# lgw-frank/Short_LDPC_Decoding_OSD

Hardware: AMD Instinct MI355X
Metric: decoded frames/sec + FER, (128,64) LDPC NMS-10+OSD-2 @ 2.5 dB (higher is better)
Workload: dtype f32; 1 GPU; nms10_osd2 -- configs[3]: NMS-10 + OSD-2, 2^20 frames over 8 GPUs = 131 072 per GPU; code=CCSDS (128,64), osd_order=2, frames_per_gpu=131072, parallelism=frame-sharded x1, rccl_ranks=1, distinct_batches_per_gpu=4, distinct_frames=524288, bytes_in_plus_out_per_rotation=545783808, nms_kernel=qc16, streams=1, osd_route=front+search

## Files before the change

### short_ldpc_decoding_osd_amd/csrc/ldpc_front.h

```cpp
#pragma once
#include "ldpc_internal.h"
#include "ldpc_wave.h"

namespace ldpc {

struct __attribute__((aligned(16))) FrontLds {
    RankLds rank;
    u64 colbuf[64];
    unsigned mask[4];
    unsigned char pi1[128];
    unsigned char rowsrc[64];
    unsigned char perm[128];
};

struct FrontResult {
    int o1, o2;
    u64 Prow;
    int ns;
};


__device__ __forceinline__ FrontResult front_device_vals(FrontLds &L, unsigned a1, unsigned a2, const u64 *__restrict__ Gcols, int lane)
{
    const float bs = bucket_scale(a1, a2);
    int r1, r2;
    bucket_ranks(L.rank, ((u64)a1 << 32) | (unsigned)(127 - lane), ((u64)a2 << 32) | (unsigned)(63 - lane), bucket_of(a1, bs),
                 bucket_of(a2, bs), lane, r1, r2);
    L.pi1[r1] = (unsigned char)lane;
    L.pi1[r2] = (unsigned char)(lane + 64);
    if (lane < 4) L.mask[lane] = 0;
    wave_fence();
    u64 C1 = Gcols[L.pi1[lane]];
    u64 C2 = Gcols[L.pi1[lane + 64]];
    int rho = lane, idx1 = lane, idx2 = lane + 64;
    const int ns = ge_columns(C1, C2, rho, idx1, idx2, lane, nullptr);
    int rankM = lane, rankL = lane;
    if (ns != 0) {
        atomicOr(&L.mask[idx1 >> 5], 1u << (idx1 & 31));
        wave_fence();
        const unsigned m[4] = {L.mask[0], L.mask[1], L.mask[2], L.mask[3]};
        rankM = below_mask(m, idx1);
        rankL = idx2 - below_mask(m, idx2);
    }
    L.perm[rankM] = L.pi1[idx1];
    L.perm[64 + rankL] = L.pi1[idx2];
    L.colbuf[rankL] = C2;
    L.rowsrc[rankM] = (unsigned char)rho;
    wave_fence();
    const u64 R = transpose64(L.colbuf[lane], lane);
    FrontResult res;
    res.Prow = shfl64(R, L.rowsrc[lane]);
    res.o1 = L.perm[lane];
    res.o2 = L.perm[64 + lane];
    res.ns = ns;
    wave_fence();
    return res;
}

__device__ __forceinline__ FrontResult front_device(FrontLds &L, const float *__restrict__ y, long long src,
                                                    const u64 *__restrict__ Gcols, int lane)
{
    return front_device_vals(L, __float_as_uint(y[src * 128 + lane]) & 0x7FFFFFFFu, __float_as_uint(y[src * 128 + 64 + lane]) & 0x7FFFFFFFu, Gcols, lane);
}


}
```

### short_ldpc_decoding_osd_amd/csrc/ldpc_osd.hip

```cpp
#include <math.h>
#include <stdlib.h>

#include "ldpc_osd_small.h"
#include "ldpc_osd_scan2.h"
#include "ldpc_osd_scan2r.h"
#include "ldpc_osd_fs.h"
#include "ldpc_osd_aux.h"
#include "ldpc_osd_state.h"

namespace ldpc {

int osd_ctx_init(ldpc_ctx *ctx)
{
    const OsdTables &t = ctx->osd_tables;
    ctx->osd_ok = false;
    if (t.n != kOsdN || t.k != kOsdK) return LDPC_OK;
    OsdState *st = new OsdState();
    ctx->osd_state = st;
    {
        int base2[127];
        auto npairs = [](int t) { return (t - 1) / 2 - (t > 63 ? t - 63 : 0) + 1; };
        for (int sidx = 0; sidx < 127; ++sidx) {
            int acc = 0;
            for (int t = sidx + 1; t <= 125; ++t) acc += npairs(t);
// ... 111 lines not shown

static unsigned grid2r(const ldpc_ctx *ctx, int64_t F) { const int64_t g = (int64_t)ctx->cu_count * 16 * 6; return (unsigned)(F < g ? F : g); }

static void launch_front(ldpc_ctx *ctx, const float *d_y, const int32_t *d_index, const int32_t *d_count, int64_t F, uint8_t *d_perm,
                         u64 *d_parity, int32_t *d_nswaps, hipStream_t s)
{
    hipLaunchKernelGGL(osd_front_kernel, dim3(frame_grid(F)), dim3(64), 0, s, d_y, d_index, d_count, (long long)F,
                       ctx->osd_tables.d_Gcols, d_perm, d_parity, d_nswaps);
}

static int need_osd(const ldpc_ctx *ctx)
{
    return ctx->osd_ok ? LDPC_OK : fail(LDPC_E_UNSUPPORTED, "OSD kernels need an (n=128, k=64) code; this one is (%d,%d)", ctx->code.n, ctx->code.k);
}

static const char *flag_name(unsigned f)
{
    if (f & LDPC_OSD_F_TABLE_SCAN) return "LDPC_OSD_F_TABLE_SCAN";
    if (f & LDPC_OSD_F_PB_BLOCK) return "LDPC_OSD_F_PB_BLOCK";
    if (f & LDPC_OSD_F_PB_REPLAY) return "LDPC_OSD_F_PB_REPLAY";
    if (f & LDPC_OSD_F_READLANE_SCAN) return "LDPC_OSD_F_READLANE_SCAN";
    return "LDPC_OSD_F_PB_FRONT_INSIDE";
}

int check_params(ldpc_ctx *ctx, const ldpc_osd_params *p, bool front_outside, const char *who)
{
    if (int rc = need_osd(ctx)) return rc;
    if (p->order < 0 || p->order > 3) return fail(LDPC_E_ARG, "%s: order %d outside 0..3", who, p->order);
    if (p->algo != LDPC_OSD_CONVENTIONAL && p->algo != LDPC_OSD_FS && p->algo != LDPC_OSD_PB)
        return fail(LDPC_E_ARG, "%s: unknown search algorithm %d", who, p->algo);
    if (p->algo == LDPC_OSD_PB && p->order < 1) return fail(LDPC_E_ARG, "%s: PB-OSD needs order >= 1", who);
    const unsigned f = (unsigned)p->flags;
    const unsigned conv = LDPC_OSD_F_TABLE_SCAN | LDPC_OSD_F_READLANE_SCAN;
    const unsigned pb = LDPC_OSD_F_PB_BLOCK | LDPC_OSD_F_PB_REPLAY | LDPC_OSD_F_PB_FRONT_INSIDE;
    if (f & ~(conv | pb)) return fail(LDPC_E_ARG, "%s: flags 0x%x are no LDPC_OSD_F_* flag", who, f & ~(conv | pb));
    if ((f & conv) && p->algo != LDPC_OSD_CONVENTIONAL)
        return fail(LDPC_E_ARG, "%s: %s needs the conventional algorithm, not %d", who, flag_name(f & conv), p->algo);
    if ((f & LDPC_OSD_F_READLANE_SCAN) && (p->order != 2 || (f & LDPC_OSD_F_TABLE_SCAN)))
        return fail(LDPC_E_ARG, "%s: LDPC_OSD_F_READLANE_SCAN needs order 2 (not %d) and no LDPC_OSD_F_TABLE_SCAN", who, p->order);
    if ((f & pb) && p->algo != LDPC_OSD_PB)
        return fail(LDPC_E_ARG, "%s: %s needs the PB algorithm, not %d", who, flag_name(f & pb), p->algo);
    if ((f & LDPC_OSD_F_PB_REPLAY) && (f & (LDPC_OSD_F_PB_BLOCK | LDPC_OSD_F_PB_FRONT_INSIDE)))
        return fail(LDPC_E_ARG, "%s: LDPC_OSD_F_PB_REPLAY excludes %s", who, flag_name(f & (LDPC_OSD_F_PB_BLOCK | LDPC_OSD_F_PB_FRONT_INSIDE)));
    if ((f & LDPC_OSD_F_PB_FRONT_INSIDE) && front_outside)
        return fail(LDPC_E_ARG, "%s: LDPC_OSD_F_PB_FRONT_INSIDE keeps the front-end results inside the PB kernels, and this call "
                    "supplies or wants them", who);
    return LDPC_OK;
}

OsdPlan select_route(const ldpc_ctx *ctx, const ldpc_osd_params *p, bool front_outside)
{
    const unsigned f = (unsigned)p->flags;
    if (p->algo == LDPC_OSD_FS) return {OsdRoute::Fs, 0};
    if (p->algo == LDPC_OSD_PB)
        return {(f & LDPC_OSD_F_PB_FRONT_INSIDE) ? OsdRoute::PbFrontInside : OsdRoute::PbStaged,
                (f & LDPC_OSD_F_PB_REPLAY) ? 2 : ((f & LDPC_OSD_F_PB_BLOCK) ? 1 : 0)};
    if (p->order != 2 || (f & LDPC_OSD_F_TABLE_SCAN)) return {OsdRoute::Table, 0};
    if ((f & LDPC_OSD_F_READLANE_SCAN) || ctx->dpp_wave_rol_dir == 0) return {OsdRoute::Search2, 0};
    return {front_outside ? OsdRoute::Search2r : OsdRoute::Fused2r, 0};
}

int osd_launch(ldpc_ctx *ctx, const float *d_y, const int32_t *d_index, const int32_t *d_count, int64_t F, const uint8_t *d_perm,
               const uint64_t *d_parity, const ldpc_osd_params *p, uint64_t *d_cw, float *d_metric, int32_t *d_best, int32_t *d_ntep,
               const uint64_t *d_label, int64_t *d_counts, hipStream_t s, bool *counted)
{
    *counted = false;
    const OsdPlan r = select_route(ctx, p, d_perm != nullptr);
    OsdState *st = state(ctx);
    const OsdTables &t = ctx->osd_tables;
    int rc;
    if ((rc = guarded_index(ctx, p, d_index, d_count, F, s, &d_index))) return rc;
    if (!d_perm && r.route != OsdRoute::Fused2r && r.route != OsdRoute::PbFrontInside) {
        StreamWs *w;
        if ((rc = stream_ws(ctx, s, F, &w))) return rc;
        launch_front(ctx, d_y, d_index, d_count, F, w->d_perm, w->d_parity, nullptr, s);
        d_perm = w->d_perm; d_parity = reinterpret_cast<const uint64_t *>(w->d_parity);
    }
    const u64 *const parity = reinterpret_cast<const u64 *>(d_parity);
    u64 *const cw = reinterpret_cast<u64 *>(d_cw);
    const u64 *const label = d_label && d_counts ? reinterpret_cast<const u64 *>(d_label) : nullptr;
    u64 *const counts = label ? reinterpret_cast<u64 *>(d_counts) : nullptr;
    const unsigned g2r = grid2r(ctx, F), g64 = frame_grid(F);
    switch (r.route) {
    case OsdRoute::Fused2r:
        hipLaunchKernelGGL(osd_fused2r_kernel, dim3(g2r), dim3(64), 0, s, d_y, d_index, d_count, (long long)F,
                           t.d_Gcols, ctx->dpp_wave_rol_dir, st->d_base2, cw, d_metric, d_best, d_ntep, label, counts);
        *counted = label != nullptr;
        break;
    case OsdRoute::Search2r:
        hipLaunchKernelGGL(osd_search2r_kernel, dim3(g2r), dim3(64), 0, s, d_y, d_index, d_count, (long long)F, d_perm, parity,
                           ctx->dpp_wave_rol_dir, st->d_base2, cw, d_metric, d_best, d_ntep, label, counts);
        *counted = label != nullptr;
        break;
    case OsdRoute::Search2:
        hipLaunchKernelGGL(osd_search2_kernel, dim3(g64), dim3(64), 0, s, d_y, d_index, d_count, (long long)F, d_perm, parity, st->d_base2,
                           cw, d_metric, d_best, d_ntep);
        break;
    case OsdRoute::Table:
        if (p->order >= 2)
            hipLaunchKernelGGL(osd_search_kernel<1>, dim3(g64), dim3(64), 0, s, d_y, d_index, d_count, (long long)F, d_perm, parity,
                               t.d_tep, (int)t.ntep[p->order], cw, d_metric, d_best, d_ntep);
        else
            hipLaunchKernelGGL(osd_search_kernel<4>, dim3(osd_grid(F)), dim3(256), 0, s, d_y, d_index, d_count, (long long)F, d_perm, parity,
                               t.d_tep, (int)t.ntep[p->order], cw, d_metric, d_best, d_ntep);
        break;
    case OsdRoute::Fs:
        hipLaunchKernelGGL(osd_fs_kernel, dim3(g64), dim3(64), 0, s, d_y, d_index, d_count, (long long)F, d_perm, parity, t.d_tep_fs,
                           fs_params(p, t), cw, d_metric, d_best, d_ntep);
        break;
    case OsdRoute::PbStaged:
        return launch_pb(ctx, d_y, d_index, d_count, F, d_perm, parity, p, r.pb_mode, false, d_cw, d_metric, d_best, d_ntep, s);
    case OsdRoute::PbFrontInside:
        return launch_pb(ctx, d_y, d_index, d_count, F, nullptr, nullptr, p, r.pb_mode, true, d_cw, d_metric, d_best, d_ntep, s);
    }
    LDPC_HIP(hipGetLastError());
    return LDPC_OK;
}

FsParams fs_params(const ldpc_osd_params *p, const OsdTables &t)
{
    FsParams fp;
    fp.order = p->order; fp.quirk = p->fs_reference_quirk != 0;
    fp.beta_term = (float)((double)p->fs_beta * (double)(t.n - t.k));
    fp.tau_e = p->fs_tau_e; fp.tau_psc = p->fs_tau_psc;
    for (int w = 0; w < 4; ++w) { fp.cls_off[w] = t.fs_off[w]; fp.cls_cnt[w] = t.fs_cnt[w]; }
    return fp;
}

}

using namespace ldpc;

extern "C" {

int ldpc_osd_reserve(ldpc_ctx *ctx, int64_t max_frames)
{
    if (!ctx || max_frames < 0) return fail(LDPC_E_ARG, "ldpc_osd_reserve: bad arguments");
    if (int rc = need_osd(ctx)) return rc;
    {
        OsdState *st = state(ctx);
        std::lock_guard<std::mutex> lock(st->mu);
        if (max_frames > st->reserve_frames) st->reserve_frames = max_frames;
    }
    StreamWs *w;
    return stream_ws(ctx, nullptr, max_frames, &w);
}

int ldpc_osd_reserve_stream(ldpc_ctx *ctx, int64_t max_frames, const ldpc_osd_params *params, void *stream)
{
    if (!ctx || max_frames < 0) return fail(LDPC_E_ARG, "ldpc_osd_reserve_stream: bad arguments");
    int rc;
    if ((rc = need_osd(ctx))) return rc;
    if (params && (rc = check_params(ctx, params, false, "ldpc_osd_reserve_stream"))) return rc;
    StreamWs *w;
    if ((rc = stream_ws(ctx, (hipStream_t)stream, max_frames, &w)) || !params) return rc;
    if (params->algo == LDPC_OSD_PB && max_frames > 0) return pb_reserve(ctx, (hipStream_t)stream, max_frames, params->order);
    return LDPC_OK;
}

int ldpc_osd_release_stream(ldpc_ctx *ctx, void *stream)
{
    if (!ctx) return fail(LDPC_E_ARG, "ldpc_osd_release_stream: null ctx");
    OsdState *st = state(ctx);
    if (!st) return LDPC_OK;
    if (stream_capturing((hipStream_t)stream)) return fail(LDPC_E_ARG, "ldpc_osd_release_stream: the stream is capturing");
    std::lock_guard<std::mutex> lock(st->mu);
    auto it = st->ws.find((hipStream_t)stream);
    if (it != st->ws.end()) { free_stream_ws(it->second); st->ws.erase(it); }
    return LDPC_OK;
}

int ldpc_osd_ge(ldpc_ctx *ctx, const uint64_t *d_rows_in, int64_t F, uint64_t *d_rows_out, uint8_t *d_swaps,
                int32_t *d_nswaps, void *stream)
{
    if (!ctx || F < 0 || (F > 0 && (!d_rows_in || !d_rows_out))) return fail(LDPC_E_ARG, "ldpc_osd_ge: bad arguments");
    if (int rc = need_osd(ctx)) return rc;
// ... 86 lines not shown
```

### short_ldpc_decoding_osd_amd/csrc/ldpc_osd_scan2r.h

```cpp
#pragma once

#include "ldpc_front.h"
#include "ldpc_osd_scan2.h"

namespace ldpc {

struct __attribute__((aligned(16))) Search2rLds {
    float lut[8][256];
    uint2 q[128];
    u64 P[64];
    __device__ __forceinline__ float *wpar() { return reinterpret_cast<float *>(q); }
    __device__ __forceinline__ u64 *cw() { return reinterpret_cast<u64 *>(q) + 32; }
};
static_assert(sizeof(Search2rLds) <= 10240, "LDS budget of the rotation scan");

__device__ __forceinline__ float cost2r(const Search2rLds &L, float mrb, u64 D)
{
    float acc = mrb;
    acc = acc + lut_byte<0>(L.lut, D); acc = acc + lut_byte<1>(L.lut, D); acc = acc + lut_byte<2>(L.lut, D); acc = acc + lut_byte<3>(L.lut, D);
    acc = acc + lut_byte<4>(L.lut, D); acc = acc + lut_byte<5>(L.lut, D); acc = acc + lut_byte<6>(L.lut, D); acc = acc + lut_byte<7>(L.lut, D);
    return acc;
}

__device__ __forceinline__ int wave_rot1(int x) { return __builtin_amdgcn_update_dpp(0, x, 0x134, 0xF, 0xF, true); }

__device__ __forceinline__ void search2r_finish_batch(const Search2rLds &L, uint2 e, bool valid, int dir, u64 d0, const int *__restrict__ base2,
                                                      float &best, int &bi, int &bj, u64 &bestD)
{
    if (!valid) return;
    const int r = (int)(e.y >> 6), l = (int)(e.y & 63), m = (l - dir * r) & 63;
    const u64 D = d0 ^ L.P[l] ^ L.P[m];
    float acc = __uint_as_float(e.x);
    acc = acc + lut_byte<2>(L.lut, D); acc = acc + lut_byte<3>(L.lut, D); acc = acc + lut_byte<4>(L.lut, D);
    acc = acc + lut_byte<5>(L.lut, D); acc = acc + lut_byte<6>(L.lut, D); acc = acc + lut_byte<7>(L.lut, D);
    if (!(acc <= best)) return;
    search2_take(acc, l < m ? l : m, l < m ? m : l, D, base2, best, bi, bj, bestD);
}

struct Scan2r {
    float m, t0, t1;
    float bound;
    int plo, wr;
    int qn;
};

__device__ __forceinline__ bool search2r_round(Search2rLds &LL, Scan2r &s, int R, unsigned dlo, float wl, int lane)
{
    float mn = 0.0f, u0 = 0.0f, u1 = 0.0f;
    if (R < 32) {
        s.plo = wave_rot1(s.plo); s.wr = wave_rot1(s.wr);
        const unsigned Dn = dlo ^ (unsigned)s.plo;
        mn = wl + __int_as_float(s.wr); u0 = lut_byte<0>(LL.lut, Dn); u1 = lut_byte<1>(LL.lut, Dn);
    }
    float acc = s.m + s.t0;
    acc = acc + s.t1;
    s.m = mn; s.t0 = u0; s.t1 = u1;
    const bool keep = (R < 32 || lane < 32) && !(acc > s.bound);
    const u64 km = __ballot(keep);
    if (!km) return false;
    if (keep) {
        const int slot = wave_lane_rank(km, (unsigned)s.qn);
        LL.q[slot] = make_uint2(__float_as_uint(acc), (unsigned)(R * 64 + lane));
    }
    s.qn += __popcll(km);
    return s.qn >= 64;
}

__device__ __forceinline__ void search2r_device(Search2rLds &LL, const SearchFrame &S, u64 Pl, float wl, int dir,
                                                const int *__restrict__ base2, int lane, float &best_out, int &rank_out,
                                                u64 &D_out, u64 &E_out)
{
    Search2rLds &L = LL;
    LL.P[lane] = Pl;
    float best;
    int bi, bj;
    u64 bestD;
    search2_start([&](float mrb, u64 D) { return cost2r(L, mrb, D); }, S.d0, Pl, wl, lane, best, bi, bj, bestD);
    const unsigned dlo = (unsigned)(S.d0 ^ Pl);
    Scan2r s;
    s.bound = wave_min_f32(best);
    s.qn = 0;
    s.plo = wave_rot1((int)(unsigned)Pl); s.wr = wave_rot1(__float_as_int(wl));
    s.m = wl + __int_as_float(s.wr);
    s.t0 = lut_byte<0>(L.lut, dlo ^ (unsigned)s.plo); s.t1 = lut_byte<1>(L.lut, dlo ^ (unsigned)s.plo);
#pragma unroll
    for (int r = 1; r <= 32; ++r) {
        if (search2r_round(LL, s, r, dlo, wl, lane)) {
            wave_fence();
            const uint2 e = LL.q[lane], rest = LL.q[64 + lane];
            s.qn -= 64;
            if (lane < s.qn) LL.q[lane] = rest;
            search2r_finish_batch(L, e, true, dir, S.d0, base2, best, bi, bj, bestD);
            s.bound = wave_min_f32(best);
            wave_fence();
        }
    }
    wave_fence();
    search2r_finish_batch(L, LL.q[lane], lane < s.qn, dir, S.d0, base2, best, bi, bj, bestD);
    wave_fence();
    int bestt = tep2_rank(bi, bj, base2);
    u64 bestE = (bi >= 0 ? 1ull << bi : 0ull) | (bj >= 0 ? 1ull << bj : 0ull);
    wave_argmin(best, bestt, bestD, bestE, lane);
    best_out = best; rank_out = bestt; D_out = bestD; E_out = bestE;
}

__device__ __forceinline__ void search2r_frame(Search2rLds &LL, int o1, int o2, u64 Pl, float y1, float y2, int dir, const int *base2,
                                               long long f, u64 lab, int lane, u64 *cw_out, float *metric_out, int *best_out,
                                               int *ntep_out, u64 *counts)
{
    SearchFrame S;
    S.o1 = o1; S.o2 = o2;
    const float w1 = __builtin_fabsf(y1), w2 = __builtin_fabsf(y2);
    LL.wpar()[lane] = w2;
    S.hm = __ballot(!(y1 > 0.0f));
    S.hp = __ballot(!(y2 > 0.0f));
    wave_fence();
    build_byte_luts<8>(LL.lut, LL.wpar(), lane);
    S.d0 = wave_xor64(((S.hm >> lane) & 1) ? Pl : 0ull) ^ S.hp;
    wave_fence();
    float best; int bestt; u64 bestD, bestE;
    search2r_device(LL, S, Pl, w1, dir, base2, lane, best, bestt, bestD, bestE);
    {
        const u64 mrb_bits = S.hm ^ bestE, par_bits = bestD ^ S.hp;
        u64 *const cw = LL.cw();
        if (lane < 2) cw[lane] = 0;
        wave_fence();
        if ((mrb_bits >> lane) & 1) atomicOr(&cw[S.o1 >> 6], 1ull << (S.o1 & 63));
        if ((par_bits >> lane) & 1) atomicOr(&cw[S.o2 >> 6], 1ull << (S.o2 & 63));
        wave_fence();
        const u64 word = lane < 2 ? cw[lane] : 0ull;
        if (lane < 2) cw_out[f * 2 + lane] = word;
        if (counts && __ballot(lane < 2 && word != lab) && lane == 0) atomicAdd(&counts[1], 1ull);
        wave_fence();
    }
    store_results(f, lane, best, bestt, 2081, metric_out, best_out, ntep_out);
}

__device__ __forceinline__ void count_up_front(u64 *__restrict__ counts, long long nframes, const int *ntep_out, int lane)
{
    if (counts && blockIdx.x == 0 && lane == 0) {
        atomicAdd(&counts[0], (u64)nframes);
        if (ntep_out) atomicAdd(&counts[2], (u64)nframes * 2081ull);
    }
}

__global__ __launch_bounds__(64) __attribute__((amdgpu_waves_per_eu(4))) void osd_search2r_kernel(const float *__restrict__ y,
        const int *__restrict__ index, const int *__restrict__ count, long long F, const unsigned char *__restrict__ perm_in,
        const u64 *__restrict__ parity_in, int dir, const int *__restrict__ base2, u64 *__restrict__ cw_out, float *__restrict__ metric_out,
        int *__restrict__ best_out, int *__restrict__ ntep_out, const u64 *__restrict__ label, u64 *__restrict__ counts)
{
    __shared__ Search2rLds LL;
    const int lane = threadIdx.x;
    const long long nframes = frame_count(count, F);
    count_up_front(counts, nframes, ntep_out, lane);
    const long long G = gridDim.x;
    long long f0 = blockIdx.x, f1 = f0 + G, f2 = f1 + G;
    int o1a = 0, o2a = 0, o1b = 0, o2b = 0;
    u64 Pa = 0, Pb = 0;
    long long srca = 0, srcb = 0;
    float y1a = 0.0f, y2a = 0.0f;
    if (f0 < nframes) {
        o1a = perm_in[f0 * 128 + lane]; o2a = perm_in[f0 * 128 + 64 + lane]; Pa = parity_in[f0 * 64 + lane];
        srca = index ? index[f0] : f0;
    }
    if (f1 < nframes) {
        o1b = perm_in[f1 * 128 + lane]; o2b = perm_in[f1 * 128 + 64 + lane]; Pb = parity_in[f1 * 64 + lane];
        srcb = index ? index[f1] : f1;
    }
    u64 laba = 0;
    if (f0 < nframes) { y1a = y[srca * 128 + o1a]; y2a = y[srca * 128 + o2a]; if (label && lane < 2) laba = label[srca * 2 + lane]; }
    while (f0 < nframes) {
        float y1b = 0.0f, y2b = 0.0f;
        u64 labb = 0;
        if (f1 < nframes) { y1b = y[srcb * 128 + o1b]; y2b = y[srcb * 128 + o2b]; if (label && lane < 2) labb = label[srcb * 2 + lane]; }
        int o1c = 0, o2c = 0;
        u64 Pc = 0;
        long long srcc = 0;
        if (f2 < nframes) {
            o1c = perm_in[f2 * 128 + lane]; o2c = perm_in[f2 * 128 + 64 + lane]; Pc = parity_in[f2 * 64 + lane];
            srcc = index ? index[f2] : f2;
        }
        search2r_frame(LL, o1a, o2a, Pa, y1a, y2a, dir, base2, f0, laba, lane, cw_out, metric_out, best_out, ntep_out, counts);
        f0 = f1; f1 = f2; f2 += G;
        o1a = o1b; o2a = o2b; Pa = Pb; srca = srcb; y1a = y1b; y2a = y2b; laba = labb;
        o1b = o1c; o2b = o2c; Pb = Pc; srcb = srcc;
    }
}

__global__ __launch_bounds__(64) __attribute__((amdgpu_waves_per_eu(4))) void osd_fused2r_kernel(const float *__restrict__ y,
        const int *__restrict__ index, const int *__restrict__ count, long long F, const u64 *__restrict__ Gcols, int dir,
        const int *__restrict__ base2, u64 *__restrict__ cw_out, float *__restrict__ metric_out, int *__restrict__ best_out,
        int *__restrict__ ntep_out, const u64 *__restrict__ label, u64 *__restrict__ counts)
{
    __shared__ Search2rLds LL;
    static_assert(sizeof(FrontLds) <= sizeof(LL.lut), "the front end works inside the LUT area");
    FrontLds &LF = *reinterpret_cast<FrontLds *>(LL.lut);
    float *const yrow = reinterpret_cast<float *>(LL.P);
    const int lane = threadIdx.x;
    long long nframes = F;
    if (count) { const long long c = *count; nframes = c < F ? c : F; }
    count_up_front(counts, nframes, ntep_out, lane);
    const long long G = gridDim.x;
    long long f0 = blockIdx.x, f1 = f0 + G, f2 = f1 + G;
    long long srca = 0, srcb = 0;
    float ya1 = 0.0f, ya2 = 0.0f;
    u64 laba = 0;
    if (f0 < nframes) srca = index ? index[f0] : f0;
    if (f1 < nframes) srcb = index ? index[f1] : f1;
    if (f0 < nframes) { ya1 = y[srca * 128 + lane]; ya2 = y[srca * 128 + 64 + lane]; if (label && lane < 2) laba = label[srca * 2 + lane]; }
    while (f0 < nframes) {
        float yb1 = 0.0f, yb2 = 0.0f;
        u64 labb = 0;
        if (f1 < nframes) { yb1 = y[srcb * 128 + lane]; yb2 = y[srcb * 128 + 64 + lane]; if (label && lane < 2) labb = label[srcb * 2 + lane]; }
        long long srcc = 0;
        if (f2 < nframes) srcc = index ? index[f2] : f2;
        yrow[lane] = ya1; yrow[64 + lane] = ya2;
        const FrontResult fr = front_device_vals(LF, __float_as_uint(ya1) & 0x7FFFFFFFu, __float_as_uint(ya2) & 0x7FFFFFFFu, Gcols, lane);
        const float y1 = yrow[fr.o1], y2 = yrow[fr.o2];
        wave_fence();
        search2r_frame(LL, fr.o1, fr.o2, fr.Prow, y1, y2, dir, base2, f0, laba, lane, cw_out, metric_out, best_out, ntep_out, counts);
        f0 = f1; f1 = f2; f2 += G;
        srca = srcb; srcb = srcc; ya1 = yb1; ya2 = yb2; laba = labb;
    }
}

}
```

### short_ldpc_decoding_osd_amd/csrc/ldpc_osd_small.h

```cpp
#pragma once

#include "ldpc_search.h"
#include "ldpc_front.h"

namespace ldpc {

__global__ __launch_bounds__(256) void osd_ge_kernel(const u64 *__restrict__ rows_in, long long F, u64 *__restrict__ rows_out,
        unsigned char *__restrict__ swaps, int *__restrict__ nswaps)
{
    const int lane = threadIdx.x & 63;
    const long long wave = (long long)blockIdx.x * 4 + (threadIdx.x >> 6);
    for (long long f = wave; f < F; f += (long long)gridDim.x * 4) {
        const u64 *src = rows_in + f * 128;
        u64 C1 = transpose64(src[lane * 2], lane);
        u64 C2 = transpose64(src[lane * 2 + 1], lane);
        int rho = lane, idx1 = lane, idx2 = lane + 64;
        const int ns = ge_columns(C1, C2, rho, idx1, idx2, lane, swaps ? swaps + f * 128 : nullptr);
        const u64 R1 = transpose64(C1, lane), R2 = transpose64(C2, lane);
        rows_out[f * 128 + lane * 2] = shfl64(R1, rho);
        rows_out[f * 128 + lane * 2 + 1] = shfl64(R2, rho);
        if (nswaps && lane == 0) nswaps[f] = ns;
    }
}

__global__ __launch_bounds__(64) void osd_front_kernel(const float *__restrict__ y, const int *__restrict__ index, const int *__restrict__ count,
        long long F, const u64 *__restrict__ Gcols, unsigned char *__restrict__ perm_out, u64 *__restrict__ parity_out, int *__restrict__ nswaps)
{
    __shared__ FrontLds L;
    const int lane = threadIdx.x;
    const long long nframes = frame_count(count, F);

    for (long long f = blockIdx.x; f < nframes; f += gridDim.x) {
        const long long src = index ? index[f] : f;
        const FrontResult res = front_device(L, y, src, Gcols, lane);
        perm_out[f * 128 + lane] = (unsigned char)res.o1;
        perm_out[f * 128 + 64 + lane] = (unsigned char)res.o2;
        parity_out[f * 64 + lane] = res.Prow;
        if (nswaps && lane == 0) nswaps[f] = res.ns;
    }
}

template <int WAVES>
__global__ __launch_bounds__(64 * WAVES) void osd_search_kernel(const float *__restrict__ y, const int *__restrict__ index,
        const int *__restrict__ count, long long F, const unsigned char *__restrict__ perm_in, const u64 *__restrict__ parity_in,
        const uchar4 *__restrict__ teps, int ntep, u64 *__restrict__ cw_out, float *__restrict__ metric_out, int *__restrict__ best_out,
        int *__restrict__ ntep_out)
{
    __shared__ SearchLds lds[WAVES];
    const int lane = threadIdx.x & 63;
    SearchLds &L = lds[WAVES == 1 ? 0 : threadIdx.x >> 6];
    const long long nframes = frame_count(count, F);
    const long long wave = (long long)blockIdx.x * WAVES + (threadIdx.x >> 6);

    for (long long f = wave; f < nframes; f += (long long)gridDim.x * WAVES) {
        const long long src = index ? index[f] : f;
        const SearchFrame S = search_prepare(L, y, src, perm_in, parity_in, f, lane);
        float best = __builtin_inff();
        int bestt = 0x7FFFFFFF;
        u64 bestD = 0, bestE = 0;
        float bound = __builtin_inff();
        int trip = 0;
        for (int t0 = 0; t0 < ntep; t0 += 64, ++trip) {
            const int t = t0 + lane;
            if (t < ntep) {
                u64 D, E;
                float mrb, c;
                tep_apply(L, teps[t], S.d0, D, E, mrb);
                if (tep_cost_bounded(L, mrb, D, bound, c) && c < best) { best = c; bestt = t; bestD = D; bestE = E; }
            }
            if ((trip & 7) == 0) bound = wave_min_f32(best);
        }
        wave_argmin(best, bestt, bestD, bestE, lane);
        search_finish(L, S, bestE, bestD, f, lane, cw_out);
        store_results(f, lane, best, bestt, ntep, metric_out, best_out, ntep_out);
    }
}

}
```

### short_ldpc_decoding_osd_amd/csrc/ldpc_pb_common.h

```cpp
#pragma once

#include "ldpc_internal.h"
#include "ldpc_wave.h"
#include "ldpc_search.h"
#include "ldpc_front.h"
#include "ldpc_osd_state.h"
#include "ldpc_pb_expf.h"

namespace ldpc {

struct PbEntry {
    float sum;
    unsigned pos;
};
constexpr int kPbLdsSlots = 512, kPbLdsChunks = 64, kPbSuper = 32;

struct __attribute__((aligned(16))) PbLds {
    double cdfA[65];
    double cdfH[65];
    float q[128];
    PbEntry fr[kPbLdsSlots];
    PbEntry cmin[kPbLdsChunks];
    PbEntry smin[kPbSuper];
};

struct PbParams {
    int order, nmax;
    int t1, t2;
    int t3, budget;
    int budget_s, budget_m;
    int budget_l, budget_xl;
    int late_min, late_maxlen, late_pct, late_div;
    int handoff_maxlen;
    float c4;
    long long cmin_off;
};

struct PbList {
    PbLds *B;
    PbEntry *spill;
    long long cmin_off;
    __device__ __forceinline__ PbEntry slot(int i) const { return i < kPbLdsSlots ? B->fr[i] : spill[i - kPbLdsSlots]; }
    __device__ __forceinline__ void set_slot(int i, PbEntry e) const { if (i < kPbLdsSlots) B->fr[i] = e; else spill[i - kPbLdsSlots] = e; }
    __device__ __forceinline__ PbEntry cmin(int c) const { return c < kPbLdsChunks ? B->cmin[c] : spill[cmin_off + c - kPbLdsChunks]; }
    __device__ __forceinline__ void set_cmin(int c, PbEntry e) const { if (c < kPbLdsChunks) B->cmin[c] = e; else spill[cmin_off + c - kPbLdsChunks] = e; }
};

__device__ __forceinline__ void argmin_si(float &s, int &idx, int lane)
{
    const float m = wave_min_f32(s);
    idx = wave_min_i32(s == m ? idx : 0x7FFFFFFF);
    s = m;
}

struct PbCoef {
    double v[64];
    constexpr PbCoef() : v() { for (int i = 0; i < 64; ++i) v[i] = (double)(64 - i) / (double)(i + 1); }
};
__constant__ PbCoef kPbCoef;

struct PbFrame {
    float spl, lrb_mean;
    double p_t_suc, p_t_pro;
};

__device__ __forceinline__ PbFrame pb_frame_setup(const float *w, float *q, double *cdfA, float c4, int order, int nmax, int lane,
                                                  float best0 = __builtin_inff(), float2 *pairs = nullptr)
{
    {
        const float q0 = 1.0f / (1.0f + det_expf(-(c4 * w[lane]))), q1 = 1.0f / (1.0f + det_expf(-(c4 * w[lane + 64])));
        q[lane] = q0;
        q[lane + 64] = q1;
        if (pairs) {
            pairs[lane] = make_float2(1.0f, q1);
            pairs[64 + lane] = make_float2(1.0f, w[lane + 64]);
            pairs[128 + lane] = make_float2(1.0f, q0);
            pairs[192 + lane] = make_float2(1.0f - q0, 0.0f);
        }
    }
    wave_fence();
    float a1, aw, at, spl;
    if (pairs) {
        const float2 *const src = pairs + 64 * (lane & 3);
        float acc = (lane & 3) == 3 ? 1.0f : 0.0f;
#pragma unroll 8
        for (int p = 0; p < 64; ++p) {
            const float2 t = src[p];
            acc = __builtin_fmaf(acc, t.x, t.y);
        }
        a1 = __int_as_float(__builtin_amdgcn_readlane(__float_as_int(acc), 0));
        aw = __int_as_float(__builtin_amdgcn_readlane(__float_as_int(acc), 1));
        at = __int_as_float(__builtin_amdgcn_readlane(__float_as_int(acc), 2));
        spl = __int_as_float(__builtin_amdgcn_readlane(__float_as_int(acc), 3));
    } else {
        const int ch = lane & 3;
        const float *src = ch == 0 ? q + 64 : (ch == 1 ? w + 64 : q);
        const bool prod = ch == 3;
        float acc = prod ? 1.0f : 0.0f;
#pragma unroll 8
        for (int p = 0; p < 64; ++p) {
            const float x = src[p];
            const float b = prod ? 1.0f - x : 1.0f, c = prod ? 0.0f : x;
            acc = __builtin_fmaf(acc, b, c);
        }
        a1 = __int_as_float(__builtin_amdgcn_readlane(__float_as_int(acc), 0));
        aw = __int_as_float(__builtin_amdgcn_readlane(__float_as_int(acc), 1));
        at = __int_as_float(__builtin_amdgcn_readlane(__float_as_int(acc), 2));
        spl = __int_as_float(__builtin_amdgcn_readlane(__float_as_int(acc), 3));
    }
    const float p1 = a1 / 64.0f, lrb_mean = aw / 64.0f, pt = at / 64.0f;
    const float bq = __builtin_floorf(best0 / lrb_mean);
    const int ncdf = bq > 0.0f ? (bq < 64.0f ? (int)bq : 64) : 0;
    double niu;
    const double coef_l = kPbCoef.v[lane];
    const auto coef = [coef_l](int i) {
        const unsigned long long b = (unsigned long long)__double_as_longlong(coef_l);
        const unsigned lo = __builtin_amdgcn_readlane((int)(unsigned)b, i), hi = __builtin_amdgcn_readlane((int)(unsigned)(b >> 32), i);
        return __longlong_as_double((long long)(((unsigned long long)hi << 32) | lo));
    };
    {
        double qq = 1.0 - (double)p1, t = qq;
        for (int s = 0; s < 6; ++s) t = t * t;
        const double ratio = (double)p1 / qq;
        double acc = t;
        if (lane == 0) cdfA[0] = acc;
#pragma unroll 2
        for (int i = 0; i < ncdf; ++i) {
            t = t * coef(i) * ratio;
            acc = acc + t;
            if (lane == 0) cdfA[i + 1] = acc;
        }
        qq = 1.0 - (double)pt; t = qq;
        for (int s = 0; s < 6; ++s) t = t * t;
// ... 145 lines not shown
```

### short_ldpc_decoding_osd_amd/csrc/ldpc_wave.h

```cpp
#pragma once

#include "ldpc_internal.h"

namespace ldpc {

typedef unsigned long long u64;

constexpr int kOsdN = 128, kOsdK = 64;

__device__ __forceinline__ long long frame_count(const int *count, long long F)
{
    long long nframes = F;
    if (count) { const long long c = *count; nframes = c < F ? c : F; }
    return nframes;
}

__device__ __forceinline__ u64 readlane64(u64 v, int lane)
{
    unsigned lo = __builtin_amdgcn_readlane((int)(unsigned)v, lane);
    unsigned hi = __builtin_amdgcn_readlane((int)(unsigned)(v >> 32), lane);
    return ((u64)hi << 32) | lo;
}

__device__ __forceinline__ u64 shfl64(u64 v, int src)
{
    unsigned lo = __shfl((int)(unsigned)v, src, 64);
    unsigned hi = __shfl((int)(unsigned)(v >> 32), src, 64);
    return ((u64)hi << 32) | lo;
}

__device__ __forceinline__ int wave_lane_rank(u64 mask, unsigned base = 0u)
{
    return (int)__builtin_amdgcn_mbcnt_hi((unsigned)(mask >> 32), __builtin_amdgcn_mbcnt_lo((unsigned)mask, base));
}

template <int CTRL, int ROWMASK>
__device__ __forceinline__ int dpp_i(int old, int x)
{
    return __builtin_amdgcn_update_dpp(old, x, CTRL, ROWMASK, 0xF, false);
}
#define LDPC_WAVE_REDUCE(v, OP)                                   \
    v = OP(v, dpp_i<0xB1, 0xF>(v, v));   \
    v = OP(v, dpp_i<0x4E, 0xF>(v, v));   \
    v = OP(v, dpp_i<0x141, 0xF>(v, v));      \
    v = OP(v, dpp_i<0x140, 0xF>(v, v));           \
    v = OP(v, dpp_i<0x142, 0xA>(ID, v));        \
    v = OP(v, dpp_i<0x143, 0xC>(ID, v));

__device__ __forceinline__ int op_xor(int a, int b) { return a ^ b; }
__device__ __forceinline__ int op_min_i(int a, int b) { return a < b ? a : b; }
__device__ __forceinline__ int op_min_f(int a, int b) { return __float_as_int(__builtin_fminf(__int_as_float(a), __int_as_float(b))); }

__device__ __forceinline__ u64 wave_xor64(u64 x)
{
    int lo = (int)(unsigned)x, hi = (int)(unsigned)(x >> 32);
    { const int ID = 0; LDPC_WAVE_REDUCE(lo, op_xor) LDPC_WAVE_REDUCE(hi, op_xor) }
    const unsigned rl = __builtin_amdgcn_readlane(lo, 63), rh = __builtin_amdgcn_readlane(hi, 63);
    return ((u64)rh << 32) | rl;
}
__device__ __forceinline__ float wave_min_f32(float x)
{
    int v = __float_as_int(x);
    { const int ID = 0x7F800000; LDPC_WAVE_REDUCE(v, op_min_f) }
    return __int_as_float(__builtin_amdgcn_readlane(v, 63));
}
__device__ __forceinline__ int wave_min_i32(int x)
{
    int v = x;
    { const int ID = 0x7FFFFFFF; LDPC_WAVE_REDUCE(v, op_min_i) }
    return __builtin_amdgcn_readlane(v, 63);
}
__device__ __forceinline__ int op_max_i(int a, int b) { return a > b ? a : b; }
__device__ __forceinline__ int wave_max_i32(int x)
{
    int v = x;
    { const int ID = (int)0x80000000; LDPC_WAVE_REDUCE(v, op_max_i) }
    return __builtin_amdgcn_readlane(v, 63);
}
__device__ __forceinline__ int op_max_f(int a, int b) { return __float_as_int(__builtin_fmaxf(__int_as_float(a), __int_as_float(b))); }
__device__ __forceinline__ int op_add_i(int a, int b) { return a + b; }
__device__ __forceinline__ float wave_max_f32(float x)
{
    int v = __float_as_int(x);
    { const int ID = (int)0xBF800000; LDPC_WAVE_REDUCE(v, op_max_f) }
    return __int_as_float(__builtin_amdgcn_readlane(v, 63));
}
__device__ __forceinline__ int wave_add_i32(int x)
{
    int v = x;
    { const int ID = 0; LDPC_WAVE_REDUCE(v, op_add_i) }
    return __builtin_amdgcn_readlane(v, 63);
}
__device__ __forceinline__ int wave_incl_add_dpp(int x)
{
    int v = x;
    v += __builtin_amdgcn_update_dpp(0, v, 0x111, 0xF, 0xF, true);
    v += __builtin_amdgcn_update_dpp(0, v, 0x112, 0xF, 0xF, true);
    v += __builtin_amdgcn_update_dpp(0, v, 0x114, 0xF, 0xF, true);
    v += __builtin_amdgcn_update_dpp(0, v, 0x118, 0xF, 0xF, true);
    v += __builtin_amdgcn_update_dpp(0, v, 0x142, 0xA, 0xF, false);
    v += __builtin_amdgcn_update_dpp(0, v, 0x143, 0xC, 0xF, false);
    return v;
}
__device__ __forceinline__ float wave_incl_addf_dpp(float x)
{
    float v = x;
    v = v + __int_as_float(__builtin_amdgcn_update_dpp(0, __float_as_int(v), 0x111, 0xF, 0xF, true));
    v = v + __int_as_float(__builtin_amdgcn_update_dpp(0, __float_as_int(v), 0x112, 0xF, 0xF, true));
    v = v + __int_as_float(__builtin_amdgcn_update_dpp(0, __float_as_int(v), 0x114, 0xF, 0xF, true));
    v = v + __int_as_float(__builtin_amdgcn_update_dpp(0, __float_as_int(v), 0x118, 0xF, 0xF, true));
    v = v + __int_as_float(__builtin_amdgcn_update_dpp(0, __float_as_int(v), 0x142, 0xA, 0xF, false));
    v = v + __int_as_float(__builtin_amdgcn_update_dpp(0, __float_as_int(v), 0x143, 0xC, 0xF, false));
    return v;
}
__device__ __forceinline__ float wave_incl_min_dpp(float x)
{
    int v = __float_as_int(x);
    const auto step = [](int v, int got) { return __float_as_int(__builtin_fminf(__int_as_float(v), __int_as_float(got))); };
    v = step(v, __builtin_amdgcn_update_dpp(v, v, 0x111, 0xF, 0xF, false));
    v = step(v, __builtin_amdgcn_update_dpp(v, v, 0x112, 0xF, 0xF, false));
    v = step(v, __builtin_amdgcn_update_dpp(v, v, 0x114, 0xF, 0xF, false));
    v = step(v, __builtin_amdgcn_update_dpp(v, v, 0x118, 0xF, 0xF, false));
    v = step(v, __builtin_amdgcn_update_dpp(v, v, 0x142, 0xA, 0xF, false));
    v = step(v, __builtin_amdgcn_update_dpp(v, v, 0x143, 0xC, 0xF, false));
    return __int_as_float(v);
}
__device__ __forceinline__ int wave_argmin_lane(float s, int idx)
{
    const float m = wave_min_f32(s);
    const int mi = wave_min_i32(s == m ? idx : 0x7FFFFFFF);
    return __builtin_ctzll(__ballot(s == m && idx == mi));
}

template <int S>
__device__ __forceinline__ u64 transpose_stage(u64 x, int lane)
{
    constexpr u64 m = S == 32 ? 0x00000000FFFFFFFFull : S == 16 ? 0x0000FFFF0000FFFFull : S == 8 ? 0x00FF00FF00FF00FFull
                    : S == 4 ? 0x0F0F0F0F0F0F0F0Full : S == 2 ? 0x3333333333333333ull : 0x5555555555555555ull;
    const u64 p = shfl64(x, lane ^ S);
    return (lane & S) ? (((p >> S) & m) | (x & ~m)) : ((x & m) | ((p & m) << S));
}

__device__ __forceinline__ u64 transpose64(u64 x, int lane)
// ... 48 lines not shown
        "2:"
        : "=&v"(m1), "=&v"(m2) : "v"(c1l), "v"(c1h), "v"(c2l), "v"(c2h), "s"(pr) : "scc");
}

__device__ __forceinline__ unsigned ge_xor_masked(unsigned c, int m, unsigned e)
{
    asm("v_bitop3_b32 %0, %0, %1, %2 bitop3:0x78" : "+v"(c) : "v"(m), "s"(e));
    return c;
}

__device__ __forceinline__ int ge_columns(u64 &C1, u64 &C2, int &rho, int &idx1, int &idx2, int lane,
                                          unsigned char *swaps )
{
    int nsw = 0;
    bool deficient = false;
    int nrho = 63 - rho;
    u64 ge_i = ~0ull;
#pragma unroll
    for (int i = 0; i < kOsdK; ++i, ge_i <<= 1) {
        u64 cj = readlane64(C1, i);
        u64 bal = ge_sign_ballot((unsigned)((cj << nrho) >> 32)) & ge_i;
        if (bal == 0) {
            const int pri = 63 - __builtin_amdgcn_readlane(nrho, i);
            const u64 b1 = __ballot((C1 >> pri) & 1) & ge_i;
            unsigned col;
            if (b1) col = __builtin_ctzll(b1);
            else {
                const u64 b2 = __ballot((C2 >> pri) & 1);
                deficient |= b2 == 0;
                col = 64 + (b2 ? __builtin_ctzll(b2) : 0);
            }
            const unsigned cl = col & 63;
            const bool lo = col < 64;
            const u64 cc1 = readlane64(C1, cl), cc2 = readlane64(C2, cl);
            const int ic1 = __builtin_amdgcn_readlane(idx1, cl), ic2 = __builtin_amdgcn_readlane(idx2, cl);
            const u64 cc = lo ? cc1 : cc2;
            const int ic = lo ? ic1 : ic2;
            const int ii = __builtin_amdgcn_readlane(idx1, i);
            const bool hit = (unsigned)lane == cl;
            C1 = (hit && lo) ? cj : C1;
            idx1 = (hit && lo) ? ii : idx1;
            C2 = (hit && !lo) ? cj : C2;
            idx2 = (hit && !lo) ? ii : idx2;
            C1 = (lane == i) ? cc : C1;
            idx1 = (lane == i) ? ic : idx1;
            if (swaps && lane == 0) { swaps[2 * nsw] = (unsigned char)i; swaps[2 * nsw + 1] = (unsigned char)col; }
            ++nsw;
            cj = readlane64(C1, i);
            bal = ge_i & (0ull - ge_i);
        }
        const int r = __builtin_ctzll(bal);
        const int npr = __builtin_amdgcn_readlane(nrho, r);
        if (r != i) {
            const int npi = __builtin_amdgcn_readlane(nrho, i);
            asm volatile("s_mov_b32 m0, %2\n\tv_writelane_b32 %0, %1, m0" : "+v"(nrho) : "s"(npr), "s"(i) : "m0");
            asm volatile("s_mov_b32 m0, %2\n\tv_writelane_b32 %0, %1, m0" : "+v"(nrho) : "s"(npi), "s"(r) : "m0");
        }
        const int pr = 63 - npr;
        const u64 e = ge_clear_bit(cj, pr);
        if (e != 0) {
            const unsigned el = (unsigned)e, eh = (unsigned)(e >> 32);
            unsigned c1l = (unsigned)C1, c1h = (unsigned)(C1 >> 32), c2l = (unsigned)C2, c2h = (unsigned)(C2 >> 32);
            int m1, m2;
            ge_row_masks(c1l, c1h, c2l, c2h, pr, m1, m2);
            c1l = ge_xor_masked(c1l, m1, el); c1h = ge_xor_masked(c1h, m1, eh);
            c2l = ge_xor_masked(c2l, m2, el); c2h = ge_xor_masked(c2h, m2, eh);
            C1 = ((u64)c1h << 32) | c1l;
            C2 = ((u64)c2h << 32) | c2l;
        }
    }
    rho = 63 - nrho;
    return deficient ? -1 : nsw;
}

struct __attribute__((aligned(16))) RankLds {
    u64 bk[256];
    int hist[64], cur[64];
    int base[64];
};

__device__ __forceinline__ float bucket_scale(unsigned a1, unsigned a2)
{
    const int m = wave_max_i32((int)(a1 > a2 ? a1 : a2));
    return 63.5f / __int_as_float(m);
}
__device__ __forceinline__ int bucket_of(unsigned a, float scale) { return (int)__builtin_fminf(__uint_as_float(a) * scale, 63.0f); }

__device__ __forceinline__ void bucket_ranks(RankLds &R, u64 k1, u64 k2, int b1, int b2, int lane, int &r1, int &r2)
{
    R.hist[lane] = 0; R.cur[lane] = 0; R.bk[128 + lane] = 0ull; R.bk[192 + lane] = 0ull;
    wave_fence();
    atomicAdd(&R.hist[b1], 1); atomicAdd(&R.hist[b2], 1);
    wave_fence();
    const int h = R.hist[lane];
    R.base[lane] = 128 - wave_incl_add_dpp(h);
    const int nmax = wave_max_i32(h);
    wave_fence();
    const int s1 = R.base[b1], s2 = R.base[b2];
    R.bk[s1 + atomicAdd(&R.cur[b1], 1)] = k1;
    R.bk[s2 + atomicAdd(&R.cur[b2], 1)] = k2;
    wave_fence();
    r1 = s1; r2 = s2;
    for (int jj = 0; jj < nmax; ++jj) { r1 += R.bk[s1 + jj] > k1; r2 += R.bk[s2 + jj] > k2; }
}

__device__ __forceinline__ void rank_gt(int &r, int a, int k)
{
    asm("v_cmp_gt_i32_e32 vcc, %2, %1\n\tv_addc_co_u32_e32 %0, vcc, 0, %0, vcc" : "+v"(r) : "v"(a), "v"(k) : "vcc");
}

__device__ __forceinline__ int below_mask(const unsigned (&m)[4], int x)
{
    int c = 0;
#pragma unroll
    for (int d = 0; d < 4; ++d) {
        const int t = x - 32 * d;
        const unsigned bm = t <= 0 ? 0u : (t >= 32 ? 0xFFFFFFFFu : ((1u << t) - 1u));
        c += __popc(m[d] & bm);
    }
    return c;
}

template <int NB>
__device__ __forceinline__ void build_byte_luts(float (*lut)[256], const float *w, int lane)
{
    const int lo5 = lane & 31, top = lane >> 5;
    const float b0 = (lo5 & 1) ? 1.0f : 0.0f, b1 = (lo5 & 2) ? 1.0f : 0.0f, b2 = (lo5 & 4) ? 1.0f : 0.0f;
    const float b3 = (lo5 & 8) ? 1.0f : 0.0f, b4 = (lo5 & 16) ? 1.0f : 0.0f, b7 = top ? 1.0f : 0.0f;
#pragma unroll
    for (int b = 0; b < NB; ++b) {
        const float4 wa = *reinterpret_cast<const float4 *>(&w[8 * b]);
        const float4 wb = *reinterpret_cast<const float4 *>(&w[8 * b + 4]);
        float base = wa.x * b0;
        base = __builtin_fmaf(wa.y, b1, base);
        base = __builtin_fmaf(wa.z, b2, base);
        base = __builtin_fmaf(wa.w, b3, base);
        base = __builtin_fmaf(wb.x, b4, base);
        const float h7 = wb.w * b7;
        lut[b][(top * 4 + 0) * 32 + lo5] = base + h7;
        lut[b][(top * 4 + 1) * 32 + lo5] = (base + wb.y) + h7;
        lut[b][(top * 4 + 2) * 32 + lo5] = (base + wb.z) + h7;
        lut[b][(top * 4 + 3) * 32 + lo5] = ((base + wb.y) + wb.z) + h7;
    }
}

template <int B>
__device__ __forceinline__ float lut_byte(const float (*lut)[256], u64 D)
{
    const unsigned word = B < 4 ? (unsigned)D : (unsigned)(D >> 32);
    unsigned off;
    if constexpr ((B & 3) == 0) asm("v_lshlrev_b32_sdwa %0, 2, %1 dst_sel:DWORD dst_unused:UNUSED_PAD src0_sel:DWORD src1_sel:BYTE_0" : "=v"(off) : "v"(word));
    else if constexpr ((B & 3) == 1) asm("v_lshlrev_b32_sdwa %0, 2, %1 dst_sel:DWORD dst_unused:UNUSED_PAD src0_sel:DWORD src1_sel:BYTE_1" : "=v"(off) : "v"(word));
    else if constexpr ((B & 3) == 2) asm("v_lshlrev_b32_sdwa %0, 2, %1 dst_sel:DWORD dst_unused:UNUSED_PAD src0_sel:DWORD src1_sel:BYTE_2" : "=v"(off) : "v"(word));
    else asm("v_lshlrev_b32_sdwa %0, 2, %1 dst_sel:DWORD dst_unused:UNUSED_PAD src0_sel:DWORD src1_sel:BYTE_3" : "=v"(off) : "v"(word));
    return *reinterpret_cast<const float *>(reinterpret_cast<const char *>(lut[B]) + off);
}

}
```

Baseline: 551.6 million frames/s.

## Micro-optimize wave reductions, rank masking, and template rotation direction

Makes the rotation direction a template parameter of the search2r and fused2r kernels, so the runtime multiply in the index computation disappears. Changes the wave min reduction to an unsigned-integer min, which matches float ordering for non-negative values, and switches the first DPP steps to bound_ctrl permutes. Rewrites below_mask with scalar popcounts, a byte perm and a bfe, replaces a division with a reciprocal, and hides the lane value from the compiler in the standalone front kernel. The unsigned min assumes non-negative metrics, and the reciprocal can differ from the exact quotient in the last bit.

```diff
diff --git a/short_ldpc_decoding_osd_amd/csrc/ldpc_front.h b/short_ldpc_decoding_osd_amd/csrc/ldpc_front.h
--- a/short_ldpc_decoding_osd_amd/csrc/ldpc_front.h
+++ b/short_ldpc_decoding_osd_amd/csrc/ldpc_front.h
@@ -20,6 +20,7 @@
 };
 
 
+template <bool GE_LANE_OPAQUE = false>
 __device__ __forceinline__ FrontResult front_device_vals(FrontLds &L, unsigned a1, unsigned a2, const u64 *__restrict__ Gcols, int lane)
 {
     const float bs = bucket_scale(a1, a2);
@@ -33,7 +34,9 @@
     u64 C1 = Gcols[L.pi1[lane]];
     u64 C2 = Gcols[L.pi1[lane + 64]];
     int rho = lane, idx1 = lane, idx2 = lane + 64;
-    const int ns = ge_columns(C1, C2, rho, idx1, idx2, lane, nullptr);
+    int ge_lane = lane;
+    if constexpr (GE_LANE_OPAQUE) asm volatile("" : "+v"(ge_lane));
+    const int ns = ge_columns(C1, C2, rho, idx1, idx2, ge_lane, nullptr);
     int rankM = lane, rankL = lane;
     if (ns != 0) {
         atomicOr(&L.mask[idx1 >> 5], 1u << (idx1 & 31));
@@ -57,10 +60,11 @@
     return res;
 }
 
+template <bool GE_LANE_OPAQUE = false>
 __device__ __forceinline__ FrontResult front_device(FrontLds &L, const float *__restrict__ y, long long src,
                                                     const u64 *__restrict__ Gcols, int lane)
 {
-    return front_device_vals(L, __float_as_uint(y[src * 128 + lane]) & 0x7FFFFFFFu, __float_as_uint(y[src * 128 + 64 + lane]) & 0x7FFFFFFFu, Gcols, lane);
+    return front_device_vals<GE_LANE_OPAQUE>(L, __float_as_uint(y[src * 128 + lane]) & 0x7FFFFFFFu, __float_as_uint(y[src * 128 + 64 + lane]) & 0x7FFFFFFFu, Gcols, lane);
 }
 
 
diff --git a/short_ldpc_decoding_osd_amd/csrc/ldpc_osd.hip b/short_ldpc_decoding_osd_amd/csrc/ldpc_osd.hip
--- a/short_ldpc_decoding_osd_amd/csrc/ldpc_osd.hip
+++ b/short_ldpc_decoding_osd_amd/csrc/ldpc_osd.hip
@@ -217,16 +217,20 @@
     u64 *const counts = label ? reinterpret_cast<u64 *>(d_counts) : nullptr;
     const unsigned g2r = grid2r(ctx, F), g64 = frame_grid(F);
     switch (r.route) {
-    case OsdRoute::Fused2r:
-        hipLaunchKernelGGL(osd_fused2r_kernel, dim3(g2r), dim3(64), 0, s, d_y, d_index, d_count, (long long)F,
-                           t.d_Gcols, ctx->dpp_wave_rol_dir, st->d_base2, cw, d_metric, d_best, d_ntep, label, counts);
+    case OsdRoute::Fused2r: {
+        const auto kernel = ctx->dpp_wave_rol_dir > 0 ? osd_fused2r_kernel<1> : osd_fused2r_kernel<-1>;
+        hipLaunchKernelGGL(kernel, dim3(g2r), dim3(64), 0, s, d_y, d_index, d_count, (long long)F, t.d_Gcols, st->d_base2, cw, d_metric,
+                           d_best, d_ntep, label, counts);
         *counted = label != nullptr;
         break;
-    case OsdRoute::Search2r:
-        hipLaunchKernelGGL(osd_search2r_kernel, dim3(g2r), dim3(64), 0, s, d_y, d_index, d_count, (long long)F, d_perm, parity,
-                           ctx->dpp_wave_rol_dir, st->d_base2, cw, d_metric, d_best, d_ntep, label, counts);
+    }
+    case OsdRoute::Search2r: {
+        const auto kernel = ctx->dpp_wave_rol_dir > 0 ? osd_search2r_kernel<1> : osd_search2r_kernel<-1>;
+        hipLaunchKernelGGL(kernel, dim3(g2r), dim3(64), 0, s, d_y, d_index, d_count, (long long)F, d_perm, parity, st->d_base2, cw, d_metric,
+                           d_best, d_ntep, label, counts);
         *counted = label != nullptr;
         break;
+    }
     case OsdRoute::Search2:
         hipLaunchKernelGGL(osd_search2_kernel, dim3(g64), dim3(64), 0, s, d_y, d_index, d_count, (long long)F, d_perm, parity, st->d_base2,
                            cw, d_metric, d_best, d_ntep);
diff --git a/short_ldpc_decoding_osd_amd/csrc/ldpc_osd_scan2r.h b/short_ldpc_decoding_osd_amd/csrc/ldpc_osd_scan2r.h
--- a/short_ldpc_decoding_osd_amd/csrc/ldpc_osd_scan2r.h
+++ b/short_ldpc_decoding_osd_amd/csrc/ldpc_osd_scan2r.h
@@ -24,11 +24,13 @@
 
 __device__ __forceinline__ int wave_rot1(int x) { return __builtin_amdgcn_update_dpp(0, x, 0x134, 0xF, 0xF, true); }
 
-__device__ __forceinline__ void search2r_finish_batch(const Search2rLds &L, uint2 e, bool valid, int dir, u64 d0, const int *__restrict__ base2,
+template <int DIR>
+__device__ __forceinline__ void search2r_finish_batch(const Search2rLds &L, uint2 e, bool valid, u64 d0, const int *__restrict__ base2,
                                                       float &best, int &bi, int &bj, u64 &bestD)
 {
+    static_assert(DIR == 1 || DIR == -1, "wave_rol:1 direction");
     if (!valid) return;
-    const int r = (int)(e.y >> 6), l = (int)(e.y & 63), m = (l - dir * r) & 63;
+    const int r = (int)(e.y >> 6), l = (int)(e.y & 63), m = (DIR > 0 ? l - r : l + r) & 63;
     const u64 D = d0 ^ L.P[l] ^ L.P[m];
     float acc = __uint_as_float(e.x);
     acc = acc + lut_byte<2>(L.lut, D); acc = acc + lut_byte<3>(L.lut, D); acc = acc + lut_byte<4>(L.lut, D);
@@ -66,7 +68,8 @@
     return s.qn >= 64;
 }
 
-__device__ __forceinline__ void search2r_device(Search2rLds &LL, const SearchFrame &S, u64 Pl, float wl, int dir,
+template <int DIR>
+__device__ __forceinline__ void search2r_device(Search2rLds &LL, const SearchFrame &S, u64 Pl, float wl,
                                                 const int *__restrict__ base2, int lane, float &best_out, int &rank_out,
                                                 u64 &D_out, u64 &E_out)
 {
@@ -90,13 +93,13 @@
             const uint2 e = LL.q[lane], rest = LL.q[64 + lane];
             s.qn -= 64;
             if (lane < s.qn) LL.q[lane] = rest;
-            search2r_finish_batch(L, e, true, dir, S.d0, base2, best, bi, bj, bestD);
+            search2r_finish_batch<DIR>(L, e, true, S.d0, base2, best, bi, bj, bestD);
             s.bound = wave_min_f32(best);
             wave_fence();
         }
     }
     wave_fence();
-    search2r_finish_batch(L, LL.q[lane], lane < s.qn, dir, S.d0, base2, best, bi, bj, bestD);
+    search2r_finish_batch<DIR>(L, LL.q[lane], lane < s.qn, S.d0, base2, best, bi, bj, bestD);
     wave_fence();
     int bestt = tep2_rank(bi, bj, base2);
     u64 bestE = (bi >= 0 ? 1ull << bi : 0ull) | (bj >= 0 ? 1ull << bj : 0ull);
@@ -104,7 +107,8 @@
     best_out = best; rank_out = bestt; D_out = bestD; E_out = bestE;
 }
 
-__device__ __forceinline__ void search2r_frame(Search2rLds &LL, int o1, int o2, u64 Pl, float y1, float y2, int dir, const int *base2,
+template <int DIR>
+__device__ __forceinline__ void search2r_frame(Search2rLds &LL, int o1, int o2, u64 Pl, float y1, float y2, const int *base2,
                                                long long f, u64 lab, int lane, u64 *cw_out, float *metric_out, int *best_out,
                                                int *ntep_out, u64 *counts)
 {
@@ -119,7 +123,7 @@
     S.d0 = wave_xor64(((S.hm >> lane) & 1) ? Pl : 0ull) ^ S.hp;
     wave_fence();
     float best; int bestt; u64 bestD, bestE;
-    search2r_device(LL, S, Pl, w1, dir, base2, lane, best, bestt, bestD, bestE);
+    search2r_device<DIR>(LL, S, Pl, w1, base2, lane, best, bestt, bestD, bestE);
     {
         const u64 mrb_bits = S.hm ^ bestE, par_bits = bestD ^ S.hp;
         u64 *const cw = LL.cw();
@@ -144,9 +148,10 @@
     }
 }
 
+template <int DIR>
 __global__ __launch_bounds__(64) __attribute__((amdgpu_waves_per_eu(4))) void osd_search2r_kernel(const float *__restrict__ y,
         const int *__restrict__ index, const int *__restrict__ count, long long F, const unsigned char *__restrict__ perm_in,
-        const u64 *__restrict__ parity_in, int dir, const int *__restrict__ base2, u64 *__restrict__ cw_out, float *__restrict__ metric_out,
+        const u64 *__restrict__ parity_in, const int *__restrict__ base2, u64 *__restrict__ cw_out, float *__restrict__ metric_out,
         int *__restrict__ best_out, int *__restrict__ ntep_out, const u64 *__restrict__ label, u64 *__restrict__ counts)
 {
     __shared__ Search2rLds LL;
@@ -180,15 +185,16 @@
             o1c = perm_in[f2 * 128 + lane]; o2c = perm_in[f2 * 128 + 64 + lane]; Pc = parity_in[f2 * 64 + lane];
             srcc = index ? index[f2] : f2;
         }
-        search2r_frame(LL, o1a, o2a, Pa, y1a, y2a, dir, base2, f0, laba, lane, cw_out, metric_out, best_out, ntep_out, counts);
+        search2r_frame<DIR>(LL, o1a, o2a, Pa, y1a, y2a, base2, f0, laba, lane, cw_out, metric_out, best_out, ntep_out, counts);
         f0 = f1; f1 = f2; f2 += G;
         o1a = o1b; o2a = o2b; Pa = Pb; srca = srcb; y1a = y1b; y2a = y2b; laba = labb;
         o1b = o1c; o2b = o2c; Pb = Pc; srcb = srcc;
     }
 }
 
+template <int DIR>
 __global__ __launch_bounds__(64) __attribute__((amdgpu_waves_per_eu(4))) void osd_fused2r_kernel(const float *__restrict__ y,
-        const int *__restrict__ index, const int *__restrict__ count, long long F, const u64 *__restrict__ Gcols, int dir,
+        const int *__restrict__ index, const int *__restrict__ count, long long F, const u64 *__restrict__ Gcols,
         const int *__restrict__ base2, u64 *__restrict__ cw_out, float *__restrict__ metric_out, int *__restrict__ best_out,
         int *__restrict__ ntep_out, const u64 *__restrict__ label, u64 *__restrict__ counts)
 {
@@ -218,7 +224,7 @@
         const FrontResult fr = front_device_vals(LF, __float_as_uint(ya1) & 0x7FFFFFFFu, __float_as_uint(ya2) & 0x7FFFFFFFu, Gcols, lane);
         const float y1 = yrow[fr.o1], y2 = yrow[fr.o2];
         wave_fence();
-        search2r_frame(LL, fr.o1, fr.o2, fr.Prow, y1, y2, dir, base2, f0, laba, lane, cw_out, metric_out, best_out, ntep_out, counts);
+        search2r_frame<DIR>(LL, fr.o1, fr.o2, fr.Prow, y1, y2, base2, f0, laba, lane, cw_out, metric_out, best_out, ntep_out, counts);
         f0 = f1; f1 = f2; f2 += G;
         srca = srcb; srcb = srcc; ya1 = yb1; ya2 = yb2; laba = labb;
     }
diff --git a/short_ldpc_decoding_osd_amd/csrc/ldpc_osd_small.h b/short_ldpc_decoding_osd_amd/csrc/ldpc_osd_small.h
--- a/short_ldpc_decoding_osd_amd/csrc/ldpc_osd_small.h
+++ b/short_ldpc_decoding_osd_amd/csrc/ldpc_osd_small.h
@@ -32,7 +32,7 @@
 
     for (long long f = blockIdx.x; f < nframes; f += gridDim.x) {
         const long long src = index ? index[f] : f;
-        const FrontResult res = front_device(L, y, src, Gcols, lane);
+        const FrontResult res = front_device<true>(L, y, src, Gcols, lane);
         perm_out[f * 128 + lane] = (unsigned char)res.o1;
         perm_out[f * 128 + 64 + lane] = (unsigned char)res.o2;
         parity_out[f * 64 + lane] = res.Prow;
diff --git a/short_ldpc_decoding_osd_amd/csrc/ldpc_pb_common.h b/short_ldpc_decoding_osd_amd/csrc/ldpc_pb_common.h
--- a/short_ldpc_decoding_osd_amd/csrc/ldpc_pb_common.h
+++ b/short_ldpc_decoding_osd_amd/csrc/ldpc_pb_common.h
@@ -48,7 +48,7 @@
 
 __device__ __forceinline__ void argmin_si(float &s, int &idx, int lane)
 {
-    const float m = wave_min_f32(s);
+    const float m = wave_min_f32_value(s);
     idx = wave_min_i32(s == m ? idx : 0x7FFFFFFF);
     s = m;
 }
diff --git a/short_ldpc_decoding_osd_amd/csrc/ldpc_wave.h b/short_ldpc_decoding_osd_amd/csrc/ldpc_wave.h
--- a/short_ldpc_decoding_osd_amd/csrc/ldpc_wave.h
+++ b/short_ldpc_decoding_osd_amd/csrc/ldpc_wave.h
@@ -39,16 +39,22 @@
 {
     return __builtin_amdgcn_update_dpp(old, x, CTRL, ROWMASK, 0xF, false);
 }
+template <int CTRL>
+__device__ __forceinline__ int dpp_perm(int x)
+{
+    return __builtin_amdgcn_update_dpp(0, x, CTRL, 0xF, 0xF, true);
+}
 #define LDPC_WAVE_REDUCE(v, OP)                                   \
-    v = OP(v, dpp_i<0xB1, 0xF>(v, v));   \
-    v = OP(v, dpp_i<0x4E, 0xF>(v, v));   \
-    v = OP(v, dpp_i<0x141, 0xF>(v, v));      \
-    v = OP(v, dpp_i<0x140, 0xF>(v, v));           \
+    v = OP(v, dpp_perm<0xB1>(v));        \
+    v = OP(v, dpp_perm<0x4E>(v));        \
+    v = OP(v, dpp_perm<0x141>(v));           \
+    v = OP(v, dpp_perm<0x140>(v));                \
     v = OP(v, dpp_i<0x142, 0xA>(ID, v));        \
     v = OP(v, dpp_i<0x143, 0xC>(ID, v));
 
 __device__ __forceinline__ int op_xor(int a, int b) { return a ^ b; }
 __device__ __forceinline__ int op_min_i(int a, int b) { return a < b ? a : b; }
+__device__ __forceinline__ int op_min_u(int a, int b) { return (unsigned)a < (unsigned)b ? a : b; }
 __device__ __forceinline__ int op_min_f(int a, int b) { return __float_as_int(__builtin_fminf(__int_as_float(a), __int_as_float(b))); }
 
 __device__ __forceinline__ u64 wave_xor64(u64 x)
@@ -59,6 +65,12 @@
     return ((u64)rh << 32) | rl;
 }
 __device__ __forceinline__ float wave_min_f32(float x)
+{
+    int v = __float_as_int(x);
+    { const int ID = -1; LDPC_WAVE_REDUCE(v, op_min_u) }
+    return __int_as_float(__builtin_amdgcn_readlane(v, 63));
+}
+__device__ __forceinline__ float wave_min_f32_value(float x)
 {
     int v = __float_as_int(x);
     { const int ID = 0x7F800000; LDPC_WAVE_REDUCE(v, op_min_f) }
@@ -273,7 +285,7 @@
 __device__ __forceinline__ float bucket_scale(unsigned a1, unsigned a2)
 {
     const int m = wave_max_i32((int)(a1 > a2 ? a1 : a2));
-    return 63.5f / __int_as_float(m);
+    return 63.5f * __builtin_amdgcn_rcpf(__int_as_float(m));
 }
 __device__ __forceinline__ int bucket_of(unsigned a, float scale) { return (int)__builtin_fminf(__uint_as_float(a) * scale, 63.0f); }
 
@@ -302,14 +314,13 @@
 
 __device__ __forceinline__ int below_mask(const unsigned (&m)[4], int x)
 {
-    int c = 0;
-#pragma unroll
-    for (int d = 0; d < 4; ++d) {
-        const int t = x - 32 * d;
-        const unsigned bm = t <= 0 ? 0u : (t >= 32 ? 0xFFFFFFFFu : ((1u << t) - 1u));
-        c += __popc(m[d] & bm);
-    }
-    return c;
+    const unsigned s0 = __builtin_amdgcn_readfirstlane(m[0]), s1 = __builtin_amdgcn_readfirstlane(m[1]);
+    const unsigned s2 = __builtin_amdgcn_readfirstlane(m[2]), s3 = __builtin_amdgcn_readfirstlane(m[3]);
+    const unsigned p1 = __popc(s0), p2 = p1 + __popc(s1), p3 = p2 + __popc(s2), p4 = p3 + __popc(s3);
+    const unsigned pre = __builtin_amdgcn_perm(p4, (p1 << 8) | (p2 << 16) | (p3 << 24), (unsigned)x >> 5);
+    const unsigned w01 = (x & 32) ? s1 : s0, w23 = (x & 32) ? s3 : s2;
+    const unsigned word = (x & 64) ? w23 : w01;
+    return (int)(pre + __popc(__builtin_amdgcn_ubfe(word, 0u, (unsigned)x & 31u)));
 }
 
 template <int NB>
```

Measured after the change: 568.6 million frames/s, median of 6. +3.1%, better.
